# eldar/deepcut-cnn

Measured on AMD Instinct MI355X. Metric: images/sec, DeeperCut ResNet-152 FCN forward (prob+loc_pred+next_pred), whole node, higher is better.
Workload: dtype f32

## Files before the change

deepcut-cnn_amd/csrc/c_api.cpp:

```cpp
#include <hip/hip_runtime_api.h>

#include <cstdio>
#include <cstring>
#include <memory>
#include <string>
#include <vector>

#include "../../include/deepcut_hip.h"
#include "net.h"

using namespace dc;


namespace {
thread_local std::string g_err;
int fail(int code, const std::string& msg) {
  g_err = msg;
  return code;
}
template <typename F>
int guard(F&& f) {
  try {
    f();
    return DC_OK;
// ... 519 lines not shown
const char* dc_net_profile_text(dc_net* net, int iters) {
  if (!net) return nullptr;
  Net* n = N(net);
  int rc = guard([&] { n->text_buf = n->profile_text(iters > 0 ? iters : 10); });
  return rc == DC_OK ? n->text_buf.c_str() : nullptr;
}

const char* dc_net_debug_info(dc_net* net) {
  if (!net) return nullptr;
  Net* n = N(net);
  int rc = guard([&] { n->text_buf = n->debug_info_text(); });
  return rc == DC_OK ? n->text_buf.c_str() : nullptr;
}

const char* dc_net_tune_report(dc_net* net) {
  if (!net) return nullptr;
  Net* n = N(net);
  int rc = guard([&] { n->text_buf = n->tune_report_text(); });
  return rc == DC_OK ? n->text_buf.c_str() : nullptr;
}
int dc_net_set_tile(dc_net* net, const char* signature, const char* tile) {
  REQUIRE(net);
  REQUIRE(signature);
  REQUIRE(tile);
  return guard([&] { N(net)->set_tile(signature, tile); });
}

int dc_conv_variant_count(void) { return dc::conv_num_variants(); }
const char* dc_conv_variant_name(int i) { return i >= 0 && i < dc::conv_num_variants() ? dc::conv_variant(i).name : nullptr; }
int dc_conv_variant_esize(int i) { return i >= 0 && i < dc::conv_num_variants() ? dc::conv_variant_esize(i) : 0; }
int dc_conv_bf16_variant_count(void) { return dc::conv_num_bf16_variants(); }
const char* dc_conv_bf16_variant_name(int i) {
  return i >= 0 && i < dc::conv_num_bf16_variants() ? dc::conv_variant(dc::kBf16Variant0 + i).name : nullptr;
}
int dc_wino_half_pack(const float* g, int cout, int cin, int rowscale, float* out, float* row_scale) {
  REQUIRE(g);
  REQUIRE(out);
  REQUIRE(row_scale);
  if (cout <= 0 || cin <= 0 || cout % 32 || cin % 16) return fail(DC_EINVAL, "dc_wino_half_pack: cout must be a multiple of 32, cin of 16");
  return guard([&] { dc::wino_half_pack_filters(g, cout, cin, rowscale != 0, out, row_scale); });
}

int dc_stream1x1_pack(const float* g, int cout, int k, float* out) {
  if (!g || !out) return fail(DC_EINVAL, "dc_stream1x1_pack: null pointer");
  if (cout <= 0 || k <= 0 || cout % 32 || k % 16) return fail(DC_EINVAL, "dc_stream1x1_pack: cout must be a multiple of 32, k of 16");
  return guard([&] { dc::stream1x1_pack_filters(g, cout, k, out); });
}

int dc_stream1x1f_pack(const float* g, int cout, int k, float* out) {
  if (!g || !out) return fail(DC_EINVAL, "dc_stream1x1f_pack: null pointer");
  if (cout <= 0 || k <= 0 || cout % 16 || k % 16) return fail(DC_EINVAL, "dc_stream1x1f_pack: cout and k must be multiples of 16");
  return guard([&] { dc::stream1x1f_pack_filters(g, cout, k, out); });
}

int dc_stem7x7_pack(const float* g, int c, float* out) {
  if (!g || !out) return fail(DC_EINVAL, "dc_stem7x7_pack: null pointer");
  if (c < 1 || c > 4) return fail(DC_EINVAL, "dc_stem7x7_pack: 1 to 4 input channels");
  return guard([&] { dc::stem7x7_pack_filters(g, c, out); });
}

namespace {
inline NetGroup* G(dc_group* g) { return reinterpret_cast<NetGroup*>(g); }
}
int dc_group_create(dc_net* const* nets, int n, dc_group** out) {
  REQUIRE(nets);
  REQUIRE(out);
// ... 145 lines not shown
```

deepcut-cnn_amd/csrc/kernels.h:

```cpp
#pragma once
#include <cstddef>
#include <cstdint>
#include <string>

namespace dc {

constexpr int kMaxTaps = 32;

void dc_magic(unsigned d, unsigned (&mg)[2]);

enum ElemKind { kElemF32 = 0, kElemF16 = 1, kElemBF16 = 2 };
inline int elem_kind_size(int kind) { return kind == kElemF32 ? 4 : 2; }
inline const char* elem_kind_name(int kind) { return kind == kElemF16 ? "f16" : kind == kElemBF16 ? "bf16" : "f32"; }

constexpr int kMaxClasses = 4;
struct ConvClass {
  int nty, ntx, dy0, ddy, x0, ddx, Ktot, x_bias;
  int OH, OW, M;
  int tiles_m;
  unsigned div_ohw[2];
  unsigned div_ow[2];
  long w_off;
  long y_off;
};

constexpr int kMaxProblems = 16;
struct ConvProblem {
  const void* x;
  void* y;
  const void* resid;
  long x_img_stride, y_img_stride;
  long w_off;
  int x_row_stride, x_rows, x_rowlen;
  int nty, ntx, dy0, ddy, x0, ddx, Ktot, x_bias;
  int OH, OW, M;
  int tiles_m;
  unsigned div_ohw[2];
  unsigned div_ow[2];
  int y_row_stride, y_pix_stride;
  int dense_x, dense_y;
  int NB;
  int pad_;
};
struct ConvMultiTable {
  int end[8][kMaxProblems];
  ConvProblem prob[kMaxProblems];
};

struct ConvGemmParams {
  int esize;
  const void* x;
  long x_img_stride;
  int x_row_stride;
  int x_rows;
  int x_rowlen;
  int sy, sx;
  int nty, ntx;
  int dy0, ddy;
  int x0, ddx;
  int klen;
  int x_bias;
  const void* w;
  int Ktot;
  int NB, OH, OW;
  int M;
  int Cout;
  void* y;
  long y_img_stride;
  int y_row_stride;
  int y_pix_stride;
  const void* resid;
  const float* scale;
  const float* shift;
  int relu;
  int sigmoid_ch;
  int xcd_on;
  int xcd_lgx;
  int tiles_m;
  unsigned div_rw[2][2];
  unsigned div_ohw[2];
  unsigned div_ow[2];
  unsigned div_tn[2];
  int tiles_n;
  long long* dbg;
  int w_TY, w_TX, w_NBY, w_NBX, w_nblk;
  unsigned w_div_nblk[2], w_div_nbyx[2], w_div_dd[2], w_div_d[2], w_div_nbx[2];
  int wide_epi;
  int vec_epi;
  int dense_x;
  int dense_y;
  int ncls;
  int mc_lgx;
  ConvClass cls[kMaxClasses];
  int nprob;
  int ekind;
};
struct ConvMultiArgs {
  ConvGemmParams p;
  ConvMultiTable t;
};
static_assert(sizeof(ConvMultiArgs) <= 4096, "HIP kernel arguments are limited to 4 KB");

struct ConvVariant {
  const char* name;
  int BM, BN, WR, WC, WK;
};
int conv_num_variants();
const ConvVariant& conv_variant(int i);
int conv_variant_bk(int i);
int conv_variant_esize(int i);
constexpr int kBf16Variant0 = 2000;
int conv_num_bf16_variants();
inline bool is_bf16_variant(int v) { return v >= kBf16Variant0 && v < kBf16Variant0 + conv_num_bf16_variants(); }
int conv_variant_ekind(int v);
bool conv_variant_exists(int v);
const int* conv_variants_of(int ekind, int* count);
int conv_variant_by_name(const char* name);
bool conv_variant_multiclass(int i);
long conv_grid(const ConvGemmParams& p, int variant);
int launch_conv_gemm(const ConvGemmParams& p, int variant, void* stream);
long prepare_conv_multi(ConvGemmParams& p, ConvMultiTable& table, int nprob, int variant);
bool conv_variant_multiproblem(int i);
int launch_conv_multi(const ConvMultiArgs& a, int variant, long grid, void* stream);

bool wino_eligible(const ConvGemmParams& p);
bool wino_same3x3(const ConvGemmParams& p);
ConvGemmParams wino_launch_params(const ConvGemmParams& p, long grid, int bty, int btx, int blocks_per_wg);
long wino_grid(const ConvGemmParams& p);
size_t wino_packed_floats(int Cout, int Cin);
void wino_pack_filters(const float* g, int Cout, int Cin, float* out);
bool wino_half_eligible(const ConvGemmParams& p);
long wino_half_grid(const ConvGemmParams& p);
size_t wino_half_packed_elems(int Cout, int Cin);
void wino_half_pack_filters(const float* g, int Cout, int Cin, bool rowscale, float* out, float* row_scale);
int launch_wino_half(const ConvGemmParams& p, void* stream);
bool stream1x1_eligible(const ConvGemmParams& p);
long stream1x1_grid(const ConvGemmParams& p);
size_t stream1x1_packed_elems(int Cout, int K);
void stream1x1_pack_filters(const float* g, int Cout, int K, float* out);
int launch_stream1x1(const ConvGemmParams& p, void* stream);
bool stream1x1f_eligible(const ConvGemmParams& p);
long stream1x1f_grid(const ConvGemmParams& p);
size_t stream1x1f_packed_elems(int Cout, int K);
void stream1x1f_pack_filters(const float* g, int Cout, int K, float* out);
int launch_stream1x1f(const ConvGemmParams& p, void* stream);
bool stem_ws_eligible(const ConvGemmParams& p);
long stem_ws_grid(const ConvGemmParams& p);
size_t stem_ws_packed_elems();
void stem_ws_pack_filters(const float* rowtap, float* out);
int launch_stem_ws(const ConvGemmParams& p, void* stream);
bool stem7x7_eligible(const ConvGemmParams& p);
long stem7x7_grid(const ConvGemmParams& p);
size_t stem7x7_packed_elems();
void stem7x7_pack_filters(const float* g, int C, float* out);
int launch_stem7x7(const ConvGemmParams& p, void* stream);
long stream1x1_prepare_multi(const ConvGemmParams& p, const ConvMultiTable& tb, int nprob);
int launch_stream1x1_multi(const ConvMultiArgs& a, void* stream);

constexpr int kWinoVariant = 1000;
constexpr int kWinoVariant16 = 1001;
constexpr int kWinoHalf = 1002;
// ... 102 lines not shown
```

deepcut-cnn_amd/csrc/kernels.hip:

```cpp
#include <hip/hip_runtime.h>

#include <algorithm>
#include <cstdlib>
#include <cstring>
#include <type_traits>
#include <vector>

#include "kernel_prims.h"
#include "kernels.h"

namespace dc {


#define DC_KARG_TOUCH(n0, n1, n2, n3, n4)                                                                                  \
  unsigned n0, n1, n2, n3, n4;                                                                                             \
  {                                                                                                                        \
    const auto* ka_ = __builtin_amdgcn_kernarg_segment_ptr();                                                              \
    asm volatile("s_load_dword %0, %5, 0x0\n\ts_load_dword %1, %5, 0x40\n\ts_load_dword %2, %5, 0x80\n\ts_load_dword %3, %5, 0xc0\n\t" \
                 "s_load_dword %4, %5, 0x100"                                                                              \
                 : "=&s"(n0), "=&s"(n1), "=&s"(n2), "=&s"(n3), "=&s"(n4)                                                     \
                 : "s"(ka_));                                                                                              \
  }
#define DC_KARG_HOLD(n0, n1, n2, n3, n4) asm volatile("" ::"s"(n0), "s"(n1), "s"(n2), "s"(n3), "s"(n4))
static_assert(sizeof(ConvGemmParams) >= 0x140, "DC_KARG_TOUCH reads five 64-byte lines of the argument block");
// ... 1266 lines not shown
    for (int qy = 0; qy < 8; ++qy) {
      int run = 0;
      for (int c = 0; c < kMaxProblems; ++c) {
        if (c < nprob && qy < (8 >> lgx)) {
          run += (int)((((long)tb.prob[c].tiles_m * (qy + 1)) >> lgy) - (((long)tb.prob[c].tiles_m * qy) >> lgy));
          tb.end[qy][c] = run;
        } else {
          tb.end[qy][c] = 0x7fffffff;
        }
      }
    }
  }
  return blk;
}

int launch_conv_multi(const ConvMultiArgs& a, int variant, long grid, void* stream) {
  if (const ConvForm* f = conv_form(variant)) return f->launch_multi ? f->launch_multi(a, stream) : (int)hipErrorInvalidValue;
  if (!dc_variant_ok(variant) || !entry_of(variant).kernel_mp || a.p.nprob < 1 || grid <= 0) return (int)hipErrorInvalidValue;
  const VariantEntry& e = entry_of(variant);
  const int nt = e.v.WR * e.v.WC * e.v.WK * 64;
  hipLaunchKernelGGL(e.kernel_mp, dim3((unsigned)grid), dim3(nt), 0, (hipStream_t)stream, a);
  return (int)hipGetLastError();
}

namespace {
constexpr int WBTY = 4, WBTX = 8, WBN = 16, WKC = 32;
constexpr int WRH = 2 * WBTY + 2, WRW = 2 * WBTX + 2;
constexpr int WPSTR = WKC + 4;
constexpr int WPITCH = 672;
constexpr int WSTAGE = WRH * WPITCH + 8;
constexpr int WNTH = 512;
static_assert(WPITCH >= WRW * WPSTR && (2 * WPITCH) % 64 == 0 && WPSTR == 36, "conflict-free ds_read_b128 layout (see above)");
static_assert(WPITCH % 4 == 0 && WPSTR % 4 == 0 && WSTAGE % 4 == 0, "16-byte units");
__device__ __forceinline__ int wino_rowbase(int row) { return row * WPITCH; }
__device__ __forceinline__ f32x2 wlo(f32x4 v) { return __builtin_shufflevector(v, v, 0, 1); }
__device__ __forceinline__ f32x2 whi(f32x4 v) { return __builtin_shufflevector(v, v, 2, 3); }
}

template <int NG>
__global__ __launch_bounds__(WNTH * NG, 4) void wino_f23_kernel(const ConvGemmParams p) {
  constexpr int NTH = WNTH * NG;
  constexpr int WNLD = (WRH * WRW * (WKC / 4) + NTH - 1) / NTH;
  const long long t_entry = (long long)__builtin_amdgcn_s_memrealtime();
  DC_KARG_TOUCH(ka0, ka1, ka2, ka3, ka4);
  __shared__ __attribute__((aligned(16))) float stage[3][WSTAGE];
  float (*part)[4][2][2][4][64] = reinterpret_cast<float (*)[4][2][2][4][64]>(&stage[0][0]);
  static_assert(sizeof(float) * NG * 4 * 2 * 2 * 4 * 64 <= sizeof(stage), "partials must fit in the staging ring");
  static_assert(2 * sizeof(stage) <= 160 * 1024, "two workgroups per CU");
  const int t = threadIdx.x, lane = t & 63, wave = t >> 6;
  auto stamp = [&](int slot) {
    if (p.dbg && lane == 0) {
      long long* d = p.dbg + ((long)blockIdx.x * (8 * NG) + wave) * 12;
      d[slot] = (long long)__builtin_readcyclecounter();
      if (slot == 0) d[8] = t_entry, d[10] = (long long)__builtin_amdgcn_s_memrealtime();
      if (slot == 7) d[9] = (long long)__builtin_amdgcn_s_memrealtime();
    }
  };
  stamp(0);
  const int C = p.klen, H = p.x_rows, W = p.x_rowlen / p.klen;
  const int d = p.ddy;
  const int NBY = p.w_NBY, NBX = p.w_NBX;
  const int nblk = p.w_nblk;
  int lb = blockIdx.x;
  if (p.xcd_on) {
    const int g8 = gridDim.x >> 3, r8 = gridDim.x & 7, q = blockIdx.x & 7;
    lb = q * g8 + min(q, r8) + (blockIdx.x >> 3);
  }
  const int nt = dc_fastdiv(lb, p.w_div_nblk), blk = lb - nt * nblk;
  const int nph = dc_fastdiv(blk, p.w_div_nbyx), brem = blk - nph * (NBY * NBX);
  const int n = dc_fastdiv(nph, p.w_div_dd), ph = nph - n * (d * d);
  const int phy = dc_fastdiv(ph, p.w_div_d), phx = ph - phy * d;
  const int by = dc_fastdiv(brem, p.w_div_nbx), bx = brem - by * NBX;
  const int oy0 = 2 * WBTY * by - 1, ox0 = 2 * WBTX * bx - 1;
  DC_KARG_HOLD(ka0, ka1, ka2, ka3, ka4);
  const int kg = lane >> 4;
  const int grp = NG == 1 ? 0 : __builtin_amdgcn_readfirstlane(wave >> 3);
  const int i = wave & 3, tf = (wave >> 2) & 1;
  const int ra = i == 0 ? 0 : (i == 2 ? 2 : 1), rb = i == 0 ? 2 : (i == 1 ? 2 : (i == 2 ? 1 : 3));
  const float sb = i == 1 ? 1.f : -1.f;
  const __amdgpu_buffer_rsrc_t xr = dc_rsrc(reinterpret_cast<const float*>(p.x) + (long)n * p.x_img_stride, 0x7fffffffu);
  const __amdgpu_buffer_rsrc_t ur = dc_rsrc(p.w, 0x7fffffffu);
  unsigned gofs[WNLD];
  int sofs[WNLD];
#pragma unroll
  for (int q = 0; q < WNLD; ++q) {
    const int e = t + q * NTH;
    const int pix = e / (WKC / 4), cq = e % (WKC / 4);
    const int py = pix / WRW, px = pix % WRW;
    const int iy = phy + d * (oy0 + py), ix = phx + d * (ox0 + px);
    const bool ok = pix < WRH * WRW && oy0 + py >= 0 && ox0 + px >= 0 && iy < H && ix < W;
    gofs[q] = ok ? (unsigned)(iy * p.x_row_stride + ix * C + cq * 4) * 4u : kOOB;
    sofs[q] = (pix < WRH * WRW ? wino_rowbase(py) + px * WPSTR + cq * 4 : WSTAGE - 8 + (t & 1) * 4) >> 2;
  }
  const int r = (lane & 15) >> 3, c = lane & 7;
  const int ofs_a = wino_rowbase(2 * (2 * tf + r) + ra) + 2 * c * WPSTR + kg * 4;
  const int ofs_b = wino_rowbase(2 * (2 * tf + r) + rb) + 2 * c * WPSTR + kg * 4;
  f32x4 acc[4];
#pragma unroll
  for (int j = 0; j < 4; ++j) acc[j] = f32x4{0.f, 0.f, 0.f, 0.f};
  const unsigned uvo = ((unsigned)((nt * 4 + i) * (C / 16)) * (4 * 64 * 4) + (unsigned)lane * 4u) * 4u;
  f32x4 g[WNLD], b[2][4], da[4], db[4];
  auto gload = [&](int K) {
#pragma unroll
    for (int q = 0; q < WNLD; ++q) g[q] = dc_bload4(xr, gofs[q], (unsigned)(K * WKC * 4));
  };
  auto sstore = [&](int buf) {
#pragma unroll
    for (int q = 0; q < WNLD; ++q) reinterpret_cast<f32x4*>(&stage[buf][0])[sofs[q]] = g[q];
  };
  auto bload = [&](int slot, int k16) {
#pragma unroll
    for (int j = 0; j < 4; ++j) b[slot][j] = dc_bload4(ur, uvo + (unsigned)j * 1024u, (unsigned)k16 * 4096u);
  };
  auto lread = [&](int buf, int h) {
#pragma unroll
    for (int c4 = 0; c4 < 4; ++c4) {
      da[c4] = *reinterpret_cast<const f32x4*>(&stage[buf][ofs_a + c4 * WPSTR + h * 16]);
      db[c4] = *reinterpret_cast<const f32x4*>(&stage[buf][ofs_b + c4 * WPSTR + h * 16]);
    }
  };
  auto compute = [&](int bslot) {
    f32x2 tl[4], th[4];
    const f32x2 sb2 = {sb, sb};
#pragma unroll
    for (int c4 = 0; c4 < 4; ++c4) {
      tl[c4] = wlo(da[c4]) + sb2 * wlo(db[c4]);
      th[c4] = whi(da[c4]) + sb2 * whi(db[c4]);
    }
    f32x2 vl[4], vh[4];
// ... 59 lines not shown
    };
    for (int K0 = 0; K0 < NS; K0 += 6) {
      step(K0, std::integral_constant<int, 0>{}, std::integral_constant<int, 0>{});
      if (K0 + 1 < NS) step(K0 + 1, std::integral_constant<int, 1>{}, std::integral_constant<int, 1>{});
      if (K0 + 2 < NS) step(K0 + 2, std::integral_constant<int, 2>{}, std::integral_constant<int, 0>{});
      if (K0 + 3 < NS) step(K0 + 3, std::integral_constant<int, 0>{}, std::integral_constant<int, 1>{});
      if (K0 + 4 < NS) step(K0 + 4, std::integral_constant<int, 1>{}, std::integral_constant<int, 0>{});
      if (K0 + 5 < NS) step(K0 + 5, std::integral_constant<int, 2>{}, std::integral_constant<int, 1>{});
    }
  }
  stamp(4);
  __syncthreads();
#pragma unroll
  for (int r4 = 0; r4 < 4; ++r4) {
    part[grp][i][0][tf][r4][lane] = acc[0][r4] + acc[1][r4] + acc[2][r4];
    part[grp][i][1][tf][r4][lane] = acc[1][r4] - acc[2][r4] - acc[3][r4];
  }
  __syncthreads();
  stamp(5);
  const int a = (wave >> 1) & 1, bq = wave & 1;
  float* yb = reinterpret_cast<float*>(p.y);
  const float* rbp = reinterpret_cast<const float*>(p.resid);
  stamp(6);
#pragma unroll
  for (int rr = 0; rr < 4 / NG; ++rr) {
    const int r4 = NG == 1 ? rr : 2 * grp + rr;
    float p0 = part[0][0][bq][tf][r4][lane], p1 = part[0][1][bq][tf][r4][lane], p2 = part[0][2][bq][tf][r4][lane], p3 = part[0][3][bq][tf][r4][lane];
    if constexpr (NG == 2) {
      p0 += part[NG - 1][0][bq][tf][r4][lane], p1 += part[NG - 1][1][bq][tf][r4][lane];
      p2 += part[NG - 1][2][bq][tf][r4][lane], p3 += part[NG - 1][3][bq][tf][r4][lane];
    }
    float v = a == 0 ? p0 + p1 + p2 : p1 - p2 - p3;
    const int q = 4 * (lane >> 4) + r4;
    const int ty = by * WBTY + 2 * tf + (q >> 3), tx = bx * WBTX + (q & 7);
    const int oy = phy + d * (2 * ty + a), ox = phx + d * (2 * tx + bq);
    if (oy < p.OH && ox < p.OW) {
      const long off = (long)n * p.y_img_stride + (long)oy * p.y_row_stride + (long)ox * p.y_pix_stride + co;
      v = v * sc + sh;
      if (rbp) v += rbp[off];
      if (p.relu) v = fmaxf(v, 0.f);
      yb[off] = v;
    }
  }
  stamp(7);
}

bool wino_same3x3(const ConvGemmParams& p) {
  const int d = p.ddy;
  if (p.nty != 3 || p.ntx != 3 || p.sy != 1 || d < 1 || d > 4 || p.dy0 != -d) return false;
  const int C = p.klen;
  if (C <= 0) return false;
  if (p.sx != C || p.ddx != d * C || p.x0 != -d * C) return false;
  if (p.x_rowlen % C != 0 || p.x_row_stride != p.x_rowlen) return false;
  return p.OH == p.x_rows && p.OW == p.x_rowlen / C;
}

ConvGemmParams wino_launch_params(const ConvGemmParams& p, long grid, int bty, int btx, int blocks_per_wg) {
  ConvGemmParams q = p;
  q.xcd_on = xcd_map_on() && grid >= 16;
  const int d = p.ddy;
  q.w_TY = ((p.OH + d - 1) / d + 1) / 2, q.w_TX = ((p.OW + d - 1) / d + 1) / 2;
  q.w_NBY = (q.w_TY + bty - 1) / bty, q.w_NBX = (q.w_TX + btx - 1) / btx;
  q.w_nblk = p.NB * d * d * q.w_NBY * q.w_NBX;
  dc_magic((unsigned)((q.w_nblk + blocks_per_wg - 1) / blocks_per_wg), q.w_div_nblk);
  dc_magic((unsigned)(q.w_NBY * q.w_NBX), q.w_div_nbyx);
  dc_magic((unsigned)(d * d), q.w_div_dd);
  dc_magic((unsigned)d, q.w_div_d);
  dc_magic((unsigned)q.w_NBX, q.w_div_nbx);
  return q;
}

bool wino_eligible(const ConvGemmParams& p) {
  if (p.esize != 4 || !wino_same3x3(p)) return false;
  const int C = p.klen;
  if (C % WKC != 0 || p.Cout % WBN != 0 || p.sigmoid_ch != 0) return false;
  if ((long long)p.x_rows * p.x_row_stride * 4 >= 0x7fffffffLL || (long long)wino_packed_floats(p.Cout, C) * 4 >= 0x7fffffffLL) return false;
  return true;
}

long wino_grid(const ConvGemmParams& p) {
  const int d = p.ddy;
  const int TY = ((p.OH + d - 1) / d + 1) / 2, TX = ((p.OW + d - 1) / d + 1) / 2;
  return (long)p.NB * d * d * ((TY + WBTY - 1) / WBTY) * ((TX + WBTX - 1) / WBTX) * (p.Cout / WBN);
}

size_t wino_packed_floats(int Cout, int Cin) { return (size_t)16 * Cout * Cin; }

void wino_pack_filters(const float* g, int Cout, int Cin, float* out) {
  static const double G[4][3] = {{1, 0, 0}, {.5, .5, .5}, {.5, -.5, .5}, {0, 0, 1}};
  for (int co = 0; co < Cout; ++co)
    for (int ci = 0; ci < Cin; ++ci) {
      const float* w = g + ((size_t)co * Cin + ci) * 9;
      double tmp[4][3], U[4][4];
      for (int a = 0; a < 4; ++a)
        for (int b = 0; b < 3; ++b) tmp[a][b] = G[a][0] * w[b] + G[a][1] * w[3 + b] + G[a][2] * w[6 + b];
      for (int a = 0; a < 4; ++a)
        for (int b = 0; b < 4; ++b) U[a][b] = tmp[a][0] * G[b][0] + tmp[a][1] * G[b][1] + tmp[a][2] * G[b][2];
      const int nt = co / 16, col = co % 16, k16 = ci / 16, kg = (ci % 16) / 4, s = ci % 4;
      const int lane = kg * 16 + col;
      for (int i = 0; i < 4; ++i)
        for (int j = 0; j < 4; ++j)
          out[(((((size_t)nt * 4 + i) * (Cin / 16) + k16) * 4 + j) * 64 + lane) * 4 + s] = (float)U[i][j];
    }
}

template <int NG>
static int launch_wino_f23(const ConvGemmParams& p, void* stream) {
  if (p.esize != 4 || !wino_eligible(p)) return (int)hipErrorInvalidValue;
  const long grid = wino_grid(p);
  if (grid <= 0) return 0;
  if (grid > 0x7fffffffL) return (int)hipErrorInvalidValue;
  hipLaunchKernelGGL(wino_f23_kernel<NG>, dim3((unsigned)grid), dim3(NG * WNTH), 0, (hipStream_t)stream, wino_launch_params(p, grid, WBTY, WBTX, 1));
  return (int)hipGetLastError();
}

static const char* const kWinoSlots[7] = {"index setup", "first loads issued", "two stages in LDS", "K loop", "partials to LDS + barrier",
                                          "inverse transform + epilogue constants", "shortcut + stores"};
static const char* const kStreamSlots[7] = {"prologue requests issued", "first stage + filters landed", "the first D steps", "the other steps",
                                            "drain", "-", "exit"};
static constexpr ConvForm kForms[kNumForms] = {
    {kWinoVariant, "wino_f23", "wino_f23<4x8x16>", kElemF32, kForm3x3, 8, kWinoSlots, wino_eligible, wino_grid, launch_wino_f23<1>,
     false, false, nullptr, nullptr, kWinoVariant16, "DC_WINOGRAD"},
    {kWinoVariant16, "wino_f23_w16", "wino_f23<4x8x16_w16>", kElemF32, kForm3x3, 16, kWinoSlots, wino_eligible, wino_grid, launch_wino_f23<2>,
     false, false, nullptr, nullptr, kWinoVariant, "DC_WINOGRAD"},
    {kWinoHalf, "wino_h23", "wino_h23<2x4x8x64>", kElemF16, kForm3x3, 8, kWinoSlots, wino_half_eligible, wino_half_grid, launch_wino_half,
     true, true, nullptr, nullptr, -1, "DC_WINOGRAD"},
    {kStreamHalf, "ws1x1", "ws1x1<32xN>", kElemF16, kForm1x1, 4, kStreamSlots, stream1x1_eligible, stream1x1_grid, launch_stream1x1,
     false, true, stream1x1_prepare_multi, launch_stream1x1_multi, -1, "DC_STREAM1X1"},
    {kStemHalf, "stem7x7", "stem7x7<8x64>", kElemF16, kFormStem, 4, kWinoSlots, stem7x7_eligible, stem7x7_grid, launch_stem7x7,
     false, false, nullptr, nullptr, -1, "DC_STEM"},
    {kStreamFloat, "ws1x1f", "ws1x1f<16xN>", kElemF32, kForm1x1, 4, kStreamSlots, stream1x1f_eligible, stream1x1f_grid, launch_stream1x1f,
     false, true, nullptr, nullptr, -1, "DC_STREAM1X1"},
    {kStemFloat, "ws7x7f", "ws7x7f<16x64>", kElemF32, kFormStem, 4, kStreamSlots, stem_ws_eligible, stem_ws_grid, launch_stem_ws,
     false, true, nullptr, nullptr, -1, "DC_STEM"},
};

static constexpr bool forms_in_variant_order() {
  for (int i = 0; i < kNumForms; ++i)
    if (kForms[i].variant != kFormVariant0 + i) return false;
  return true;
}
static_assert(forms_in_variant_order(), "row i of kForms is variant kFormVariant0 + i");

const ConvForm* conv_form(int variant) {
  return variant >= kFormVariant0 && variant < kFormVariant0 + kNumForms ? &kForms[variant - kFormVariant0] : nullptr;
// ... 682 lines not shown
```

deepcut-cnn_amd/csrc/net_lower.cpp:

```cpp
#include "net_internal.h"

namespace dc {

namespace {
struct LOp {
  enum Kind { CONV, DECONV, POOL, ELT, CROP } kind = CONV;
  std::vector<int> lids;
  int in = -1, in2 = -1, out = -1;
  int wl = -1;
  std::vector<int> wls;
  std::vector<double> a, b;
  int sigmoid_ch = -1;
  bool relu = false, sigmoid = false;
  int oh = 0, ow = 0;
  bool fused_crop = false;
  bool dead = false;
};

double variant_cost(const ConvGemmParams& p, int v) {
  const ConvVariant& cv = conv_variant(v);
  int bk = conv_variant_bk(v);
  int FM = cv.BM / cv.WR / 32, FN = cv.BN / cv.WC / 32;
  const double wps = cv.WR * cv.WC * cv.WK / 4.0;
  double wgs = (double)conv_grid(p, v);
// ... 412 lines not shown
        segs.push_back({0, l.cg.Ktot});
      for (const Seg& sg : segs)
        if (sg.off + (size_t)OC * sg.K > Wv.host.size())
          throw DcError(DC_EINVAL, "launch '" + l.label + "': filter image of " + std::to_string(Wv.host.size()) + " elements is smaller than " +
                                       std::to_string(OC) + " rows of " + std::to_string(sg.K));
      Wv.row_scale.assign(OC, 1.f);
      for (int c = 0; c < OC; ++c) {
        float mx = 0.f;
        for (const Seg& sg : segs) {
          const float* r = Wv.host.data() + sg.off + (size_t)c * sg.K;
          for (int k = 0; k < sg.K; ++k) mx = std::max(mx, std::fabs(r[k]));
        }
        if (!(mx > 0.f) || !std::isfinite(mx)) continue;
        int k = 13 - std::ilogb(mx);
        k = std::max(-60, std::min(60, k));
        if (k == 0) continue;
        const float f = std::ldexp(1.f, k);
        for (const Seg& sg : segs) {
          float* r = Wv.host.data() + sg.off + (size_t)c * sg.K;
          for (int q = 0; q < sg.K; ++q) r[q] *= f;
        }
        Wv.row_scale[c] = std::ldexp(1.f, -k);
      }
    }
    std::shared_ptr<DevVec> rs = l.w;
    char wkey[40];
    std::snprintf(wkey, sizeof wkey, "%p", (void*)l.w.get());
    l.scale = get_vec(std::string("ha:") + wkey + ":" + std::to_string(op.lids.front()) + ":" + std::to_string(op.lids.size()), [&](std::vector<float>& h) {
      h.resize(OC);
      for (int c = 0; c < OC; ++c) h[c] = (float)((op.a.empty() ? 1.0 : op.a[c]) * (double)rs->row_scale[c]);
    });
  };
  const int wino_mode = env_int("DC_WINOGRAD", -1);
  const int stem_mode = env_int("DC_STEM", -1);
  const int stream_mode = env_int("DC_STREAM1X1", -1);
  auto choose_variant = [&](Launch& l, int kgcd) {
    int best = -1;
    double bc = 0;
    const bool mc = l.cg.ncls > 1;
    for (int ci = 0; ci < ncand; ++ci) {
      const int v = cand[ci];
      if (!tile_takes_k(v, kgcd, l.row_tap) || (mc && !conv_variant_multiclass(v))) continue;
      if (force_variant >= 0 && v != force_variant) continue;
      double c = variant_cost(l.cg, v);
      if (best < 0 || c < bc) best = v, bc = c;
    }
    if (best < 0)
      for (int ci = 0; ci < ncand; ++ci) {
        const int v = cand[ci];
        if (!tile_takes_k(v, kgcd, l.row_tap) || (mc && !conv_variant_multiclass(v))) continue;
        double c = variant_cost(l.cg, v);
        if (best < 0 || c < bc) best = v, bc = c;
      }
    if (best < 0) throw DcError(DC_EUNSUP, "launch '" + l.label + "': no tile variant takes K segments of " + std::to_string(kgcd) + " elements");
    l.set_variant(best);
  };
  auto offer_form = [&](Launch& l, int v) {
    if (env_int(conv_form(v)->env, -1) >= 1 && (force_variant < 0 || conv_form(force_variant))) l.set_variant(v);
  };

  const int head_split = env_int("DC_HEAD_SPLIT", 0);
  auto push_split = [&](Launch&& l, int kgcd) {
    const int OC = l.cg.Cout;
    const bool want = head_split == 1;
    const int c0 = OC / 128 * 128;
    if (!want || OC < 256 || c0 == OC || OC - c0 > 64 || force_variant >= 0) {
// ... 104 lines not shown
          const int taps = c.kh * c.kw;
          int cbase = 0;
          for (int ml : members) {
            const float* w = layers[ml].params[0]->st->host_ptr();
            const int cm = layers[ml].conv.num_output;
            for (int co = 0; co < cm; ++co)
              for (int ci = 0; ci < C; ++ci) {
                const float* src = w + ((size_t)co * C + ci) * taps;
                float* dst = h.data() + (size_t)(cbase + co) * g.Ktot + ci;
                for (int tp = 0; tp < taps; ++tp) dst[(size_t)tp * CP] = src[tp];
              }
            cbase += cm;
          }
        });
      }
      g.NB = N;
      g.OH = OHt;
      g.OW = OWt;
      g.M = N * OHt * OWt;
      g.Cout = OC;
      g.y_img_stride = (long)OHt * OWt * OCP;
      g.y_row_stride = OWt * OCP;
      g.y_pix_stride = OCP;
      g.relu = op.relu;
      g.sigmoid_ch = op.sigmoid ? OC : 0;
      affine_vecs(op, l, OC);
      l.flops = 2.0 * g.M * (double)OC * C * c.kh * c.kw;
      plan_flops += l.flops;
      l.w->as_half = dtype == kElemF16;
      l.w->as_bf16 = dtype == kElemBF16;
          half_row_scale(l, op, OC);
      choose_variant(l, kgcd);
      if (!rowtap && wino_mode != 0 && op.wls.empty() && wino_eligible(g) && dtype == kElemF32) {
        l.form_w = get_vec(dkey + "wino:" + std::to_string(op.wl), [&](std::vector<float>& h) {
          h.assign(wino_packed_floats(c.num_output, C), 0.f);
          wino_pack_filters(L.params[0]->st->host_ptr(), c.num_output, C, h.data());
        });
        offer_form(l, wino_mode == 2 ? kWinoVariant16 : kWinoVariant);
      } else if (!rowtap && wino_mode != 0 && op.wls.empty() && dtype == kElemF16 && op.in2 < 0 && wino_half_eligible(g)) {
        std::vector<float> rs_made;
        l.form_w = get_vec(dkey + "wino:" + std::to_string(op.wl), [&](std::vector<float>& h) {
          h.assign(wino_half_packed_elems(c.num_output, C), 0.f);
          rs_made.assign(c.num_output, 1.f);
          wino_half_pack_filters(L.params[0]->st->host_ptr(), c.num_output, C, half_rowscale, h.data(), rs_made.data());
        });
        if (!rs_made.empty()) l.form_w->row_scale = std::move(rs_made);
        l.form_w->as_half = true;
        std::shared_ptr<DevVec> ws = l.form_w;
        char wkey[40];
        std::snprintf(wkey, sizeof wkey, "%p", (void*)ws.get());
        l.form_scale = get_vec(std::string("hwa:") + wkey + ":" + std::to_string(op.lids.front()) + ":" + std::to_string(op.lids.size()), [&](std::vector<float>& h) {
          h.resize(OC);
          for (int q = 0; q < OC; ++q) h[q] = (float)((op.a.empty() ? 1.0 : op.a[q]) * 4.0 * (double)(ws->row_scale.empty() ? 1.f : ws->row_scale[q]));
        });
        offer_form(l, kWinoHalf);
      } else if (!rowtap && stream_mode != 0 && op.wls.empty() && dtype == kElemF16 && g.klen == C && g.Ktot == C && stream1x1_eligible(g)) {
        std::shared_ptr<DevVec> direct = l.w;
        l.form_w = get_vec(dkey + "ws:" + std::to_string(op.wl), [&](std::vector<float>& h) {
          const float* src = L.params[0]->st->host_ptr();
          std::vector<float> scaled((size_t)OC * C);
          for (int co = 0; co < OC; ++co) {
            const float f = direct->row_scale.empty() ? 1.f : 1.f / direct->row_scale[co];
            for (int k = 0; k < C; ++k) scaled[(size_t)co * C + k] = src[(size_t)co * C + k] * f;
          }
          h.assign(stream1x1_packed_elems(OC, C), 0.f);
          stream1x1_pack_filters(scaled.data(), OC, C, h.data());
// ... 338 lines not shown
```

deepcut-cnn_amd/python/caffe/__init__.py:

```python
from .pycaffe import Net, NetGroup, Comm, Blob, Layer, choose_streams, pinned_empty, lpt_schedule, set_mode_cpu, set_mode_gpu, set_device, device_count, canvas_size, check_boxes, member_canvas, conv_variants, conv_variants_bf16, wino_half_pack, stream1x1_pack, stream1x1f_pack, stem7x7_pack, lib_path
from .pycaffe import TRAIN, TEST, DeepcutError

__version__ = "1.0.0-rc3+deepcut_hip"
```

deepcut-cnn_amd/python/caffe/pycaffe.py:

```python
import ctypes as C
import os
import sys
from collections import OrderedDict

import numpy as np

TRAIN = 0
TEST = 1

_HERE = os.path.dirname(os.path.abspath(__file__))
_LIB_CANDIDATES = [
    os.environ.get("DEEPCUT_HIP_LIB", ""),
    os.path.normpath(os.path.join(_HERE, "..", "..", "lib", "libdeepcut_hip.so")),
]


class DeepcutError(RuntimeError):

    def __init__(self, code, msg):
        RuntimeError.__init__(self, msg)
        self.code = code


def lib_path():
# ... 83 lines not shown
        "dc_group_destroy": (ci, [vp]),
        "dc_group_size": (ci, [vp]),
        "dc_group_set_lanes": (ci, [vp, ci]),
        "dc_group_forward_batch": (ci, [vp, C.POINTER(vp), C.POINTER(ci), C.POINTER(ci), C.POINTER(ci), ci, C.POINTER(vp), C.POINTER(vp),
                                        C.POINTER(vp), vp]),
        "dc_group_forward_images": (ci, [vp, C.POINTER(vp), C.POINTER(ci), C.POINTER(ci), C.POINTER(ci), C.POINTER(C.c_double), ci,
                                         C.POINTER(vp), C.POINTER(vp), C.POINTER(vp), C.POINTER(vp), vp]),
        "dc_group_forward_boxes": (ci, [vp, vp, ci, ci, ci, vp, vp, ci, C.POINTER(C.c_double), ci, ci, C.POINTER(vp), C.POINTER(vp),
                                        C.POINTER(vp), C.POINTER(vp), vp]),
        "dc_group_plan_text": (cp, [vp]),
        "dc_group_profile_text": (cp, [vp, ci]),
        "dc_group_tune_report": (cp, [vp]),
        "dc_group_set_tile": (ci, [vp, cp, cp]),
        "dc_group_stats": (ci, [vp, C.POINTER(C.c_longlong), ci]),
        "dc_group_flops": (ci, [vp, C.POINTER(C.c_double)]),
        "dc_net_forward_host_async": (ci, [vp, vp, ci, ci, ci, vp, vp, vp]),
        "dc_host_alloc": (ci, [C.c_size_t, C.POINTER(vp)]),
        "dc_host_free": (ci, [vp]),
        "dc_nets_choose_streams": (ci, [C.POINTER(vp), ci, ci, ci, C.POINTER(C.c_double), C.POINTER(C.c_double)]),
        "dc_net_stream": (ci, [vp, C.POINTER(vp)]),
        "dc_comm_create": (ci, [ci, C.POINTER(ci), ci, C.POINTER(vp)]),
        "dc_comm_destroy": (ci, [vp]),
        "dc_comm_transport": (ci, [vp]),
        "dc_forward_batch": (ci, [vp, C.POINTER(vp), ci, C.POINTER(vp), C.POINTER(ci * 2), ci, C.POINTER(vp), C.POINTER(vp), C.POINTER(vp)]),
        "dc_comm_item_executor": (ci, [vp, ci]),
        "dc_comm_root_maps": (ci, [vp, ci, C.POINTER(vp), C.POINTER(vp), C.POINTER(vp), C.POINTER(ci)]),
        "dc_lpt_schedule": (ci, [C.POINTER(C.c_double), ci, ci, C.POINTER(ci)]),
        "dc_conv_variant_count": (ci, []),
        "dc_conv_variant_name": (cp, [ci]),
        "dc_conv_variant_esize": (ci, [ci]),
        "dc_conv_bf16_variant_count": (ci, []),
        "dc_conv_bf16_variant_name": (cp, [ci]),
        "dc_wino_half_pack": (ci, [C.c_void_p, ci, ci, ci, C.c_void_p, C.c_void_p]),
        "dc_stream1x1_pack": (ci, [C.c_void_p, ci, ci, C.c_void_p]),
        "dc_stem7x7_pack": (ci, [C.c_void_p, ci, C.c_void_p]),
        "dc_stream1x1f_pack": (ci, [C.c_void_p, ci, ci, C.c_void_p]),
    }
    for name, (res, args) in sig.items():
        fn = getattr(lib, name)
        fn.restype = res
        fn.argtypes = args
    return lib, sorted(sig)


_lib, EXPORTED_SYMBOLS = _load()


def _check(rc):
    if rc != 0:
        raise DeepcutError(rc, (_lib.dc_last_error() or b"").decode())


def set_mode_cpu():
    _check(_lib.dc_set_mode(0))


def set_mode_gpu():
    _check(_lib.dc_set_mode(1))


def set_device(device_id):
    _check(_lib.dc_set_device(int(device_id)))


def device_count():
    return _lib.dc_device_count()
# ... 2 lines not shown
_DTYPES = {"f32": 0, "float32": 0, "f16": 1, "float16": 1, "bf16": 2, "bfloat16": 2}


def conv_variants():
    return [((_lib.dc_conv_variant_name(i) or b"").decode(), _lib.dc_conv_variant_esize(i)) for i in range(_lib.dc_conv_variant_count())]


def conv_variants_bf16():
    return [(_lib.dc_conv_bf16_variant_name(i) or b"").decode() for i in range(_lib.dc_conv_bf16_variant_count())]


def stream1x1_pack(g):
    g = np.ascontiguousarray(g, np.float32)
    cout, k = g.shape[0], int(np.prod(g.shape[1:]))
    out = np.empty((cout // 32, k // 16, 64, 8), np.float32)
    _check(_lib.dc_stream1x1_pack(g.ctypes.data_as(C.c_void_p), cout, k, out.ctypes.data_as(C.c_void_p)))
    return out


def stream1x1f_pack(g):
    g = np.ascontiguousarray(g, np.float32)
    cout, k = g.shape[0], int(np.prod(g.shape[1:]))
    out = np.empty((cout // 16, k // 16, 64, 4), np.float32)
    _check(_lib.dc_stream1x1f_pack(g.ctypes.data_as(C.c_void_p), cout, k, out.ctypes.data_as(C.c_void_p)))
    return out


def stem7x7_pack(g):
    g = np.ascontiguousarray(g, np.float32)
    if g.ndim != 4 or g.shape[0] != 64 or g.shape[2:] != (7, 7):
        raise ValueError("stem7x7_pack: g must be [64, c, 7, 7]")
    out = np.empty((2, 7, 2, 64, 8), np.float32)
    _check(_lib.dc_stem7x7_pack(g.ctypes.data_as(C.c_void_p), g.shape[1], out.ctypes.data_as(C.c_void_p)))
    return out


def wino_half_pack(g, rowscale=True):
    g = np.ascontiguousarray(g, dtype=np.float32)
    cout, cin = g.shape[:2]
    out = np.empty((cout // 32, 4, cin // 16, 4, 64, 8), np.float32)
    rs = np.empty(cout, np.float32)
    _check(_lib.dc_wino_half_pack(g.ctypes.data_as(C.c_void_p), cout, cin, 1 if rowscale else 0, out.ctypes.data_as(C.c_void_p), rs.ctypes.data_as(C.c_void_p)))
    return out, rs


def canvas_size(height, width, scale):
    h, w = C.c_int(), C.c_int()
    _check(_lib.dc_image_canvas_size(int(height), int(width), float(scale), C.byref(h), C.byref(w)))
    return h.value, w.value


def member_canvas(side, pyramid_scale):
    return int(np.ceil(float(side) * float(pyramid_scale) / 8) * 8)


def check_boxes(image_shape, boxes, scales=1.0, canvas=None):
    h, w = int(image_shape[0]), int(image_shape[1])
    b = np.asarray(boxes)
    if b.size == 0:
        b = b.reshape(0, 4)
    if b.ndim != 2 or b.shape[1] != 4:
        raise ValueError("boxes must be an n x 4 array of (x0, y0, x1, y1), got shape %s" % (b.shape,))
    if not np.issubdtype(b.dtype, np.integer):
        if not (np.isfinite(b).all() and (b == np.round(b)).all()):
            raise ValueError("box corners must be whole pixels")
    b = np.ascontiguousarray(b, dtype=np.int32)
# ... 822 lines not shown
```

include/deepcut_hip.h:

```cpp
#ifndef DEEPCUT_HIP_H_
#define DEEPCUT_HIP_H_

#include <stddef.h>
#include <stdint.h>

#ifdef __cplusplus
extern "C" {
#endif

#define DC_OK 0
#define DC_EINVAL (-1)
#define DC_EIO (-2)
#define DC_ESHAPE (-3)
#define DC_EUNSUP (-4)
#define DC_EDEVICE (-5)
#define DC_ENOCPU (-6)

#define DC_MODE_CPU 0
#define DC_MODE_GPU 1
#define DC_PHASE_TRAIN 0
#define DC_PHASE_TEST 1

#define DC_OPT_FUSE 1
#define DC_OPT_HIPGRAPH 2
// ... 84 lines not shown
int dc_net_forward_boxes(dc_net* net, const unsigned char* image, int height, int width, int is_device, const int* boxes, const double* scales,
                         int n, int canvas_h, int canvas_w, float* prob, float* loc_pred, float* next_pred, double* pose, void* stream);

int dc_net_detect_parts(dc_net* net, double scale, float threshold, int radius, int max_det, int* counts, double* dets);
int dc_net_decode_pairwise(dc_net* net, double scale, int ndet, const int* detections, const double* mean,
                           const double* stdev, double* out);


int dc_net_flops(dc_net* net, double* flops);
int dc_net_num_launches(dc_net* net);
#define DC_STAT_LOWERINGS 0
#define DC_STAT_GRAPH_INSTANTIATIONS 1
#define DC_STAT_PLAN_HITS 2
#define DC_STAT_AUTOTUNE_RUNS 3
#define DC_STAT_BUFFER_GROWTHS 4
#define DC_STAT_REPACKS 5
#define DC_STAT_CACHED_PLANS 6
#define DC_NUM_STATS 7
int dc_net_stats(dc_net* net, long long* out, int n);
int dc_net_reserve(dc_net* net, int n, int h, int w);
int dc_net_device(dc_net* net);
const char* dc_net_plan_text(dc_net* net);
const char* dc_net_profile_text(dc_net* net, int iters);
const char* dc_net_debug_info(dc_net* net);
const char* dc_net_tune_report(dc_net* net);
int dc_net_set_tile(dc_net* net, const char* signature, const char* tile);
int dc_conv_variant_count(void);
const char* dc_conv_variant_name(int i);
int dc_conv_variant_esize(int i);
int dc_conv_bf16_variant_count(void);
const char* dc_conv_bf16_variant_name(int i);
int dc_wino_half_pack(const float* g, int cout, int cin, int rowscale, float* out, float* row_scale);

int dc_stream1x1_pack(const float* g, int cout, int k, float* out);
int dc_stem7x7_pack(const float* g, int c, float* out);
int dc_stream1x1f_pack(const float* g, int cout, int k, float* out);

typedef struct dc_group dc_group;
int dc_group_create(dc_net* const* nets, int n, dc_group** out);
int dc_group_destroy(dc_group* group);
int dc_group_size(dc_group* group);
int dc_group_set_lanes(dc_group* group, int lanes);
int dc_group_forward_batch(dc_group* group, const float* const* inputs, const int* n, const int* h, const int* w, int is_device,
                           float* const* prob, float* const* loc_pred, float* const* next_pred, void* stream);
int dc_group_forward_images(dc_group* group, const unsigned char* const* images, const int* n, const int* height, const int* width,
                            const double* scale, int is_device, float* const* prob, float* const* loc_pred, float* const* next_pred,
                            double* const* pose, void* stream);
int dc_group_forward_boxes(dc_group* group, const unsigned char* image, int height, int width, int is_device, const int* boxes,
                           const double* scales, int n, const double* pyramid_scales, int canvas_h, int canvas_w, float* const* prob,
                           float* const* loc_pred, float* const* next_pred, double* const* pose, void* stream);
const char* dc_group_plan_text(dc_group* group);
const char* dc_group_profile_text(dc_group* group, int iters);
const char* dc_group_tune_report(dc_group* group);
int dc_group_set_tile(dc_group* group, const char* signature, const char* tile);
#define DC_GSTAT_MERGES 0
#define DC_GSTAT_GRAPH_INSTANTIATIONS 1
#define DC_GSTAT_AUTOTUNE_RUNS 2
#define DC_GSTAT_PLAN_HITS 3
#define DC_GSTAT_LAUNCHES 4
#define DC_GSTAT_MULTI_LAUNCHES 5
#define DC_GSTAT_LANES 6
#define DC_NUM_GSTATS 7
int dc_group_stats(dc_group* group, long long* out, int n);
int dc_group_flops(dc_group* group, double* out);

#define DC_COMM_AUTO 0
// ... 17 lines not shown
```

Before: 518.4.

## Cover Winograd F(2,3) tile grid with mixed 4x8/8x4 block regions

The Winograd 3x3 kernel now covers the output tile grid with up to four rectangular regions. Each region uses either the original 4x8 block geometry or a new 8x4 geometry with its own LDS pitch, and a host-side search picks the split that needs the fewest blocks. This cuts wasted padded blocks on feature maps whose tile dimensions don't divide evenly, which shrinks the grid. In exchange the kernel pays for region lookup, geometry-dependent index math and extra kernarg loads, and it can be disabled with DC_WINO_COVER=0.

```diff
diff --git a/deepcut-cnn_amd/csrc/c_api.cpp b/deepcut-cnn_amd/csrc/c_api.cpp
--- a/deepcut-cnn_amd/csrc/c_api.cpp
+++ b/deepcut-cnn_amd/csrc/c_api.cpp
@@ -575,6 +575,22 @@
 int dc_conv_bf16_variant_count(void) { return dc::conv_num_bf16_variants(); }
 const char* dc_conv_bf16_variant_name(int i) {
   return i >= 0 && i < dc::conv_num_bf16_variants() ? dc::conv_variant(dc::kBf16Variant0 + i).name : nullptr;
+}
+int dc_wino_cover(int ty, int tx, int smallest, int* blocks, int cap) {
+  if (ty <= 0 || tx <= 0 || cap < 0 || (cap > 0 && !blocks)) {
+    fail(DC_EINVAL, "dc_wino_cover: ty, tx must be positive, blocks must hold cap entries");
+    return -1;
+  }
+  const dc::WinoCover cv = dc::wino_cover(ty, tx, smallest != 0);
+  int n = 0;
+  for (int k = 0; k < cv.nreg; ++k) {
+    const dc::WinoRegion& g = cv.reg[k];
+    const int bty = g.geo == dc::kWinoGeo8x4 ? 8 : 4, btx = g.geo == dc::kWinoGeo8x4 ? 4 : 8;
+    for (int by = 0; by < g.nby; ++by)
+      for (int bx = 0; bx < g.nbx; ++bx, ++n)
+        if (n < cap) blocks[4 * n] = g.ty0 + by * bty, blocks[4 * n + 1] = g.tx0 + bx * btx, blocks[4 * n + 2] = bty, blocks[4 * n + 3] = btx;
+  }
+  return n;
 }
 int dc_wino_half_pack(const float* g, int cout, int cin, int rowscale, float* out, float* row_scale) {
   REQUIRE(g);
diff --git a/deepcut-cnn_amd/csrc/kernels.h b/deepcut-cnn_amd/csrc/kernels.h
--- a/deepcut-cnn_amd/csrc/kernels.h
+++ b/deepcut-cnn_amd/csrc/kernels.h
@@ -45,6 +45,17 @@
 struct ConvMultiTable {
   int end[8][kMaxProblems];
   ConvProblem prob[kMaxProblems];
+};
+
+struct WinoRegionArg {
+  int first;
+  int ty0, tx0, geo, nbx;
+  unsigned div_nbx[2];
+  int pad_;
+};
+constexpr int kWinoMaxRegions = 4;
+struct alignas(64) WinoCoverArgs {
+  WinoRegionArg r[kWinoMaxRegions];
 };
 
 struct ConvGemmParams {
@@ -94,6 +105,8 @@
   ConvClass cls[kMaxClasses];
   int nprob;
   int ekind;
+  int w_cover_off;
+  WinoCoverArgs w_cov;
 };
 struct ConvMultiArgs {
   ConvGemmParams p;
@@ -127,6 +140,16 @@
 bool wino_same3x3(const ConvGemmParams& p);
 ConvGemmParams wino_launch_params(const ConvGemmParams& p, long grid, int bty, int btx, int blocks_per_wg);
 long wino_grid(const ConvGemmParams& p);
+constexpr int kWinoGeo4x8 = 0, kWinoGeo8x4 = 1;
+struct WinoRegion {
+  int ty0, tx0, ty1, tx1;
+  int geo, nby, nbx, first;
+};
+struct WinoCover {
+  int nreg, nblk;
+  WinoRegion reg[kWinoMaxRegions];
+};
+WinoCover wino_cover(int ty, int tx, bool smallest);
 size_t wino_packed_floats(int Cout, int Cin);
 void wino_pack_filters(const float* g, int Cout, int Cin, float* out);
 bool wino_half_eligible(const ConvGemmParams& p);
diff --git a/deepcut-cnn_amd/csrc/kernels.hip b/deepcut-cnn_amd/csrc/kernels.hip
--- a/deepcut-cnn_amd/csrc/kernels.hip
+++ b/deepcut-cnn_amd/csrc/kernels.hip
@@ -1322,7 +1322,12 @@
 constexpr int WNTH = 512;
 static_assert(WPITCH >= WRW * WPSTR && (2 * WPITCH) % 64 == 0 && WPSTR == 36, "conflict-free ds_read_b128 layout (see above)");
 static_assert(WPITCH % 4 == 0 && WPSTR % 4 == 0 && WSTAGE % 4 == 0, "16-byte units");
-__device__ __forceinline__ int wino_rowbase(int row) { return row * WPITCH; }
+constexpr int WBTY2 = 8, WBTX2 = 4;
+constexpr int WRH2 = 2 * WBTY2 + 2, WRW2 = 2 * WBTX2 + 2;
+constexpr int WPITCH2 = 368;
+static_assert(WBTY2 * WBTX2 == WBTY * WBTX && WRH2 * WRW2 == WRH * WRW, "both geometries: 32 tiles, 180 staged pixels");
+static_assert(WPITCH2 >= WRW2 * WPSTR && (2 * WPITCH2) % 64 == 32 && WPITCH2 % 4 == 0, "conflict-free ds_read_b128 layout of the 8x4 block");
+static_assert(WRH2 * WPITCH2 + 8 <= WSTAGE, "the 8x4 block fits the stage of the 4x8 block (dump slot included)");
 __device__ __forceinline__ f32x2 wlo(f32x4 v) { return __builtin_shufflevector(v, v, 0, 1); }
 __device__ __forceinline__ f32x2 whi(f32x4 v) { return __builtin_shufflevector(v, v, 2, 3); }
 }
@@ -1333,6 +1338,10 @@
   constexpr int WNLD = (WRH * WRW * (WKC / 4) + NTH - 1) / NTH;
   const long long t_entry = (long long)__builtin_amdgcn_s_memrealtime();
   DC_KARG_TOUCH(ka0, ka1, ka2, ka3, ka4);
+  unsigned ka5, ka6;
+  asm volatile("s_load_dword %0, %2, %3\n\ts_load_dword %1, %2, %4"
+               : "=&s"(ka5), "=&s"(ka6)
+               : "s"(__builtin_amdgcn_kernarg_segment_ptr()), "i"(offsetof(ConvGemmParams, w_cov)), "i"(offsetof(ConvGemmParams, w_cov) + 64));
   __shared__ __attribute__((aligned(16))) float stage[3][WSTAGE];
   float (*part)[4][2][2][4][64] = reinterpret_cast<float (*)[4][2][2][4][64]>(&stage[0][0]);
   static_assert(sizeof(float) * NG * 4 * 2 * 2 * 4 * 64 <= sizeof(stage), "partials must fit in the staging ring");
@@ -1349,7 +1358,6 @@
   stamp(0);
   const int C = p.klen, H = p.x_rows, W = p.x_rowlen / p.klen;
   const int d = p.ddy;
-  const int NBY = p.w_NBY, NBX = p.w_NBX;
   const int nblk = p.w_nblk;
   int lb = blockIdx.x;
   if (p.xcd_on) {
@@ -1357,12 +1365,21 @@
     lb = q * g8 + min(q, r8) + (blockIdx.x >> 3);
   }
   const int nt = dc_fastdiv(lb, p.w_div_nblk), blk = lb - nt * nblk;
-  const int nph = dc_fastdiv(blk, p.w_div_nbyx), brem = blk - nph * (NBY * NBX);
+  const int nph = dc_fastdiv(blk, p.w_div_nbyx), brem = blk - nph * p.w_NBY;
   const int n = dc_fastdiv(nph, p.w_div_dd), ph = nph - n * (d * d);
   const int phy = dc_fastdiv(ph, p.w_div_d), phx = ph - phy * d;
-  const int by = dc_fastdiv(brem, p.w_div_nbx), bx = brem - by * NBX;
-  const int oy0 = 2 * WBTY * by - 1, ox0 = 2 * WBTX * bx - 1;
+  WinoRegionArg rg = p.w_cov.r[0];
+#pragma unroll
+  for (int k = 1; k < kWinoMaxRegions; ++k)
+    if (brem >= p.w_cov.r[k].first) rg = p.w_cov.r[k];
+  const int bi = brem - rg.first;
+  const int by = dc_fastdiv(bi, rg.div_nbx), bx = bi - by * rg.nbx;
+  const bool g84 = rg.geo == kWinoGeo8x4;
+  const int ty0 = rg.ty0 + by * (g84 ? WBTY2 : WBTY), tx0 = rg.tx0 + bx * (g84 ? WBTX2 : WBTX);
+  const int oy0 = 2 * ty0 - 1, ox0 = 2 * tx0 - 1;
+  const int pitch = g84 ? WPITCH2 : WPITCH;
   DC_KARG_HOLD(ka0, ka1, ka2, ka3, ka4);
+  asm volatile("" ::"s"(ka5), "s"(ka6));
   const int kg = lane >> 4;
   const int grp = NG == 1 ? 0 : __builtin_amdgcn_readfirstlane(wave >> 3);
   const int i = wave & 3, tf = (wave >> 2) & 1;
@@ -1376,15 +1393,15 @@
   for (int q = 0; q < WNLD; ++q) {
     const int e = t + q * NTH;
     const int pix = e / (WKC / 4), cq = e % (WKC / 4);
-    const int py = pix / WRW, px = pix % WRW;
+    const int py = g84 ? pix / WRW2 : pix / WRW, px = pix - py * (g84 ? WRW2 : WRW);
     const int iy = phy + d * (oy0 + py), ix = phx + d * (ox0 + px);
     const bool ok = pix < WRH * WRW && oy0 + py >= 0 && ox0 + px >= 0 && iy < H && ix < W;
     gofs[q] = ok ? (unsigned)(iy * p.x_row_stride + ix * C + cq * 4) * 4u : kOOB;
-    sofs[q] = (pix < WRH * WRW ? wino_rowbase(py) + px * WPSTR + cq * 4 : WSTAGE - 8 + (t & 1) * 4) >> 2;
-  }
-  const int r = (lane & 15) >> 3, c = lane & 7;
-  const int ofs_a = wino_rowbase(2 * (2 * tf + r) + ra) + 2 * c * WPSTR + kg * 4;
-  const int ofs_b = wino_rowbase(2 * (2 * tf + r) + rb) + 2 * c * WPSTR + kg * 4;
+    sofs[q] = (pix < WRH * WRW ? py * pitch + px * WPSTR + cq * 4 : WSTAGE - 8 + (t & 1) * 4) >> 2;
+  }
+  const int r = g84 ? 4 * tf + ((lane & 15) >> 2) : 2 * tf + ((lane & 15) >> 3), c = g84 ? lane & 3 : lane & 7;
+  const int ofs_a = (2 * r + ra) * pitch + 2 * c * WPSTR + kg * 4;
+  const int ofs_b = (2 * r + rb) * pitch + 2 * c * WPSTR + kg * 4;
   f32x4 acc[4];
 #pragma unroll
   for (int j = 0; j < 4; ++j) acc[j] = f32x4{0.f, 0.f, 0.f, 0.f};
@@ -1510,7 +1527,7 @@
     }
     float v = a == 0 ? p0 + p1 + p2 : p1 - p2 - p3;
     const int q = 4 * (lane >> 4) + r4;
-    const int ty = by * WBTY + 2 * tf + (q >> 3), tx = bx * WBTX + (q & 7);
+    const int ty = ty0 + (g84 ? 4 * tf + (q >> 2) : 2 * tf + (q >> 3)), tx = tx0 + (g84 ? q & 3 : q & 7);
     const int oy = phy + d * (2 * ty + a), ox = phx + d * (2 * tx + bq);
     if (oy < p.OH && ox < p.OW) {
       const long off = (long)n * p.y_img_stride + (long)oy * p.y_row_stride + (long)ox * p.y_pix_stride + co;
@@ -1556,10 +1573,51 @@
   return true;
 }
 
+WinoCover wino_cover(int ty, int tx, bool smallest) {
+  WinoCover best{};
+  if (ty <= 0 || tx <= 0) return best;
+  struct Rect {
+    int y0, x0, y1, x1, geo, n;
+  };
+  auto tile = [&](int y0, int x0, int y1, int x1) {
+    const int h = y1 - y0, w = x1 - x0;
+    const int n48 = ((h + WBTY - 1) / WBTY) * ((w + WBTX - 1) / WBTX), n84 = ((h + WBTY2 - 1) / WBTY2) * ((w + WBTX2 - 1) / WBTX2);
+    return smallest && n84 < n48 ? Rect{y0, x0, y1, x1, kWinoGeo8x4, n84} : Rect{y0, x0, y1, x1, kWinoGeo4x8, n48};
+  };
+  auto band = [&](int y0, int y1, Rect(&out)[2]) {
+    out[0] = tile(y0, 0, y1, tx), out[1] = Rect{0, 0, 0, 0, 0, 0};
+    int n = out[0].n;
+    for (int xs = 8; smallest && xs < tx; xs += 8) {
+      const Rect a = tile(y0, 0, y1, xs), b = tile(y0, xs, y1, tx);
+      if (a.n + b.n < n) n = a.n + b.n, out[0] = a, out[1] = b;
+    }
+    return n;
+  };
+  Rect pick[4], cur[2][2];
+  int nbest = band(0, ty, cur[0]);
+  pick[0] = cur[0][0], pick[1] = cur[0][1], pick[2] = pick[3] = Rect{0, 0, 0, 0, 0, 0};
+  for (int ys = 8; smallest && ys < ty; ys += 8) {
+    const int n = band(0, ys, cur[0]) + band(ys, ty, cur[1]);
+    if (n < nbest) nbest = n, pick[0] = cur[0][0], pick[1] = cur[0][1], pick[2] = cur[1][0], pick[3] = cur[1][1];
+  }
+  for (const Rect& r : pick) {
+    if (r.n == 0) continue;
+    const int bty = r.geo == kWinoGeo8x4 ? WBTY2 : WBTY, btx = r.geo == kWinoGeo8x4 ? WBTX2 : WBTX;
+    WinoRegion& g = best.reg[best.nreg++];
+    g = WinoRegion{r.y0, r.x0, r.y1, r.x1, r.geo, (r.y1 - r.y0 + bty - 1) / bty, (r.x1 - r.x0 + btx - 1) / btx, best.nblk};
+    best.nblk += g.nby * g.nbx;
+  }
+  return best;
+}
+
+static WinoCover wino_cover_of(const ConvGemmParams& p) {
+  const int d = p.ddy;
+  return wino_cover(((p.OH + d - 1) / d + 1) / 2, ((p.OW + d - 1) / d + 1) / 2, !p.w_cover_off);
+}
+
 long wino_grid(const ConvGemmParams& p) {
   const int d = p.ddy;
-  const int TY = ((p.OH + d - 1) / d + 1) / 2, TX = ((p.OW + d - 1) / d + 1) / 2;
-  return (long)p.NB * d * d * ((TY + WBTY - 1) / WBTY) * ((TX + WBTX - 1) / WBTX) * (p.Cout / WBN);
+  return (long)p.NB * d * d * wino_cover_of(p).nblk * (p.Cout / WBN);
 }
 
 size_t wino_packed_floats(int Cout, int Cin) { return (size_t)16 * Cout * Cin; }
@@ -1588,7 +1646,23 @@
   const long grid = wino_grid(p);
   if (grid <= 0) return 0;
   if (grid > 0x7fffffffL) return (int)hipErrorInvalidValue;
-  hipLaunchKernelGGL(wino_f23_kernel<NG>, dim3((unsigned)grid), dim3(NG * WNTH), 0, (hipStream_t)stream, wino_launch_params(p, grid, WBTY, WBTX, 1));
+  ConvGemmParams q = wino_launch_params(p, grid, WBTY, WBTX, 1);
+  const WinoCover cv = wino_cover_of(p);
+  const int d = p.ddy;
+  q.w_NBY = cv.nblk, q.w_NBX = 1;
+  q.w_nblk = p.NB * d * d * cv.nblk;
+  dc_magic((unsigned)q.w_nblk, q.w_div_nblk);
+  dc_magic((unsigned)cv.nblk, q.w_div_nbyx);
+  for (int k = 0; k < kWinoMaxRegions; ++k) {
+    WinoRegionArg& a = q.w_cov.r[k];
+    a = WinoRegionArg{};
+    a.first = 0x7fffffff;
+    if (k >= cv.nreg) continue;
+    const WinoRegion& g = cv.reg[k];
+    a.first = g.first, a.ty0 = g.ty0, a.tx0 = g.tx0, a.geo = g.geo, a.nbx = g.nbx;
+    dc_magic((unsigned)g.nbx, a.div_nbx);
+  }
+  hipLaunchKernelGGL(wino_f23_kernel<NG>, dim3((unsigned)grid), dim3(NG * WNTH), 0, (hipStream_t)stream, q);
   return (int)hipGetLastError();
 }
 
diff --git a/deepcut-cnn_amd/csrc/net_lower.cpp b/deepcut-cnn_amd/csrc/net_lower.cpp
--- a/deepcut-cnn_amd/csrc/net_lower.cpp
+++ b/deepcut-cnn_amd/csrc/net_lower.cpp
@@ -468,6 +468,7 @@
     });
   };
   const int wino_mode = env_int("DC_WINOGRAD", -1);
+  const bool wino_cover_off = env_int("DC_WINO_COVER", 1) == 0;
   const int stem_mode = env_int("DC_STEM", -1);
   const int stream_mode = env_int("DC_STREAM1X1", -1);
   auto choose_variant = [&](Launch& l, int kgcd) {
@@ -638,6 +639,7 @@
           half_row_scale(l, op, OC);
       choose_variant(l, kgcd);
       if (!rowtap && wino_mode != 0 && op.wls.empty() && wino_eligible(g) && dtype == kElemF32) {
+        g.w_cover_off = wino_cover_off;
         l.form_w = get_vec(dkey + "wino:" + std::to_string(op.wl), [&](std::vector<float>& h) {
           h.assign(wino_packed_floats(c.num_output, C), 0.f);
           wino_pack_filters(L.params[0]->st->host_ptr(), c.num_output, C, h.data());
diff --git a/deepcut-cnn_amd/python/caffe/__init__.py b/deepcut-cnn_amd/python/caffe/__init__.py
--- a/deepcut-cnn_amd/python/caffe/__init__.py
+++ b/deepcut-cnn_amd/python/caffe/__init__.py
@@ -1,4 +1,4 @@
-from .pycaffe import Net, NetGroup, Comm, Blob, Layer, choose_streams, pinned_empty, lpt_schedule, set_mode_cpu, set_mode_gpu, set_device, device_count, canvas_size, check_boxes, member_canvas, conv_variants, conv_variants_bf16, wino_half_pack, stream1x1_pack, stream1x1f_pack, stem7x7_pack, lib_path
+from .pycaffe import Net, NetGroup, Comm, Blob, Layer, choose_streams, pinned_empty, lpt_schedule, set_mode_cpu, set_mode_gpu, set_device, device_count, canvas_size, check_boxes, member_canvas, conv_variants, conv_variants_bf16, wino_half_pack, wino_cover, stream1x1_pack, stream1x1f_pack, stem7x7_pack, lib_path
 from .pycaffe import TRAIN, TEST, DeepcutError
 
 __version__ = "1.0.0-rc3+deepcut_hip"
diff --git a/deepcut-cnn_amd/python/caffe/pycaffe.py b/deepcut-cnn_amd/python/caffe/pycaffe.py
--- a/deepcut-cnn_amd/python/caffe/pycaffe.py
+++ b/deepcut-cnn_amd/python/caffe/pycaffe.py
@@ -139,6 +139,7 @@
         "dc_conv_bf16_variant_count": (ci, []),
         "dc_conv_bf16_variant_name": (cp, [ci]),
         "dc_wino_half_pack": (ci, [C.c_void_p, ci, ci, ci, C.c_void_p, C.c_void_p]),
+        "dc_wino_cover": (ci, [ci, ci, ci, C.c_void_p, ci]),
         "dc_stream1x1_pack": (ci, [C.c_void_p, ci, ci, C.c_void_p]),
         "dc_stem7x7_pack": (ci, [C.c_void_p, ci, C.c_void_p]),
         "dc_stream1x1f_pack": (ci, [C.c_void_p, ci, ci, C.c_void_p]),
@@ -207,6 +208,16 @@
         raise ValueError("stem7x7_pack: g must be [64, c, 7, 7]")
     out = np.empty((2, 7, 2, 64, 8), np.float32)
     _check(_lib.dc_stem7x7_pack(g.ctypes.data_as(C.c_void_p), g.shape[1], out.ctypes.data_as(C.c_void_p)))
+    return out
+
+
+def wino_cover(ty, tx, smallest=True):
+    n = _lib.dc_wino_cover(ty, tx, 1 if smallest else 0, None, 0)
+    if n < 0:
+        raise DeepcutError(1, (_lib.dc_last_error() or b"").decode())
+    out = np.zeros((n, 4), np.int32)
+    if _lib.dc_wino_cover(ty, tx, 1 if smallest else 0, out.ctypes.data_as(C.c_void_p), n) != n:
+        raise RuntimeError("dc_wino_cover changed its mind")
     return out
 
 
diff --git a/include/deepcut_hip.h b/include/deepcut_hip.h
--- a/include/deepcut_hip.h
+++ b/include/deepcut_hip.h
@@ -140,6 +140,8 @@
 const char* dc_conv_bf16_variant_name(int i);
 int dc_wino_half_pack(const float* g, int cout, int cin, int rowscale, float* out, float* row_scale);
 
+int dc_wino_cover(int ty, int tx, int smallest, int* blocks, int cap);
+
 int dc_stream1x1_pack(const float* g, int cout, int k, float* out);
 int dc_stem7x7_pack(const float* g, int c, float* out);
 int dc_stream1x1f_pack(const float* g, int cout, int k, float* out);
```

Result: faster. 523.8 (median of 6 runs) (+1.0%).
